# FeMTTU/femus

Hardware: AMD Instinct MI355X
Metric: assembled DOFs/sec + V-cycle SpMV GB/s (% HBM peak), 3D Poisson Q2 (higher is better)
Workload: dtype f64

## Files before the change

femus_amd/capi.py:

```python
import ctypes
import numpy as np
from ._lib import load_library

GEOM = {"hex": 0, "quad": 1, "line": 2, "tri": 3, "tet": 4, "wedge": 5}
FE = {"linear": 0, "serendipity": 1, "biquadratic": 2, "constant": 3, "pwlinear": 4}
GAUSS_ORDER = {"zero": 0, "first": 0, "second": 1, "third": 1, "fourth": 2, "fifth": 2,
               "sixth": 3, "seventh": 3, "eighth": 4, "ninth": 4}
OUTER = {"preonly": 0, "richardson": 1, "gmres": 2, "cg": 3, "fgmres": 4}
SMOOTH_JACOBI, SMOOTH_GS_COLOR, SMOOTH_VANKA, SMOOTH_SOR, SMOOTH_ILU0, SMOOTH_IDENTITY, SMOOTH_LU, SMOOTH_ASM = 0, 1, 2, 3, 4, 5, 6, 7


class FemusHipError(RuntimeError):
    pass


def _chk(rc):
    if rc != 0:
        raise FemusHipError(load_library().fh_last_error().decode())


def _i32(a):
    return np.ascontiguousarray(a, dtype=np.int32)


# ... 927 lines not shown
        a, g = ctypes.c_int(), ctypes.c_int()
        _chk(self.L.fh_assembler_affine_count(self.h, ctypes.byref(a), ctypes.byref(g)))
        return a.value, g.value

    def last_path(self):
        v = ctypes.c_int()
        _chk(self.L.fh_assembler_last_path(self.h, ctypes.byref(v)))
        return {1: "fused", 2: "two-pass"}.get(v.value)

    def fused_info(self):
        a, n, r = ctypes.c_int(), ctypes.c_int(), ctypes.c_int()
        pe = ctypes.c_int64()
        _chk(self.L.fh_assembler_fused_info(self.h, ctypes.byref(a), ctypes.byref(n), ctypes.byref(pe), ctypes.byref(r)))
        cs, ce = ctypes.c_int(), ctypes.c_int64()
        _chk(self.L.fh_assembler_carry_info(self.h, ctypes.byref(cs), ctypes.byref(ce)))
        return {"active": bool(a.value), "clusters": n.value, "partial_entries": pe.value, "second_pass_rows": r.value,
                "clusters_per_super": cs.value, "carried_entries": ce.value}

    def assemble_expr(self, A, res, sol, expr, scale=1.0):
        _chk(self.L.fh_assemble_poisson_expr(self.h, None if sol is None else sol.h, expr.h, float(scale), A.h, res.h))

    def element_matrices(self, sol=None, source_kind=0, params=(1.0,)):
        p = _f64(list(params) + [0.0] * (4 - len(params)))
        K, F = np.empty((self.nel, self.nc, self.nc)), np.empty((self.nel, self.nc))
        _chk(self.L.fh_element_matrices_poisson(self.h, None if sol is None else sol.h, int(source_kind), _p(p), _p(K), _p(F)))
        return K, F

    def info(self, colors=True):
        nco, by, fl = ctypes.c_int(), ctypes.c_int64(), ctypes.c_double()
        _chk(self.L.fh_assembler_info(self.h, ctypes.byref(nco) if colors else None, ctypes.byref(by), ctypes.byref(fl)))
        return {"ncolors": nco.value if colors else None, "algorithmic_bytes": by.value, "flops": fl.value}

# ... 400 lines not shown
```

femus_amd/csrc/fh_assemble.hip:

```cpp
#include "fh_internal.h"
#include "fh_fe.h"
#include "fh_expr_device.h"
#include <algorithm>

struct SfTab { double L[3][4], D[3][4]; };

struct fh_assembler_s {
  fh_ctx_t ctx = nullptr;
  int geom = 0, fe = 0, order = 0, dim = 3, nc = 27, ng = 64, nloc = 27;
  int nel = 0, nnode = 0, ndof = 0;
  int ncolors = 0;
  std::vector<int> color_ptr;
  int* d_color_elems = nullptr;
  int* d_elem_dof = nullptr;
  double* d_coords = nullptr;
  double* d_w = nullptr;
  double* d_phi = nullptr;
  double* d_dphi = nullptr;
  int* d_emap = nullptr;
  int* d_iota = nullptr;
  int ncp = 28;
  int* d_adj_ptr = nullptr;
  int* d_adj_ei = nullptr;
  unsigned char* d_rowmap = nullptr;
// ... 14 lines not shown
  bool kbuf_valid = false;
  bool rows_used_since = false;
  int last_path = 0;
  int cl_ncl = 0, cl_nm = 0, cl_ns = 0, cl_nprow = 0;
  int cl_sup_shift = 0;
  int cl_walk_shift = 0;
  size_t cl_ncarried = 0;
  size_t cl_npart = 0;
  unsigned* d_cl_sinfo = nullptr;
  void *d_cl_dtab = nullptr, *d_cl_fblk = nullptr, *d_cl_oblk = nullptr;
  int *d_cl_vdst = nullptr, *d_cl_fdst = nullptr;
  unsigned long long* d_cl_vdst64 = nullptr;
  double* cl_val_base = nullptr;
  unsigned char *d_cl_map = nullptr, *d_cl_pmap = nullptr;
  unsigned char* d_cl_mapb = nullptr;
  unsigned short* d_cl_gtab = nullptr;
  bool cl_all_rows = false;
  bool macro_valid = false;
  uint64_t macro_uid = 0;
  uint64_t macro_val_gen = 0;
  double* d_Pbuf = nullptr;
  int* d_cl_prow = nullptr;
  unsigned* d_cl_pstart = nullptr;
  int last_source_kind = 0;
  double last_params[2] = {1.0, 0.0};
  int *d_aff_elems = nullptr, *d_gen_elems = nullptr;
  int n_aff = 0, n_gen = 0;
  double *d_Mab = nullptr, *d_mphi = nullptr;
  double *d_mfT = nullptr, *d_mfPhi = nullptr;
  double* d_mfSFc = nullptr;
// ... 1587 lines not shown
static_assert(CL_ZC < (1 << 16), "cluster kernel: 16-bit double indices of the address blocks");
static_assert(cl_lds_bytes() <= 160 * 1024, "cluster kernel: LDS budget");
static_assert((CL_TAB % 2) == 0 && (CL_UVS % 2) == 0, "cluster kernel: 16-byte alignment of the wave regions");

struct ClParams {
  int ncl, ns, nm;
  int sup_shift;
  const uint2* dtab;
  const uint4* fblk;
  const uint4* oblk;
  const unsigned* sinfo;
  const unsigned long long* vdst;
  const int* fdst;
  const uint4* map;
  const uint4* mapb;
  double* Pbuf;
  double* res;
  unsigned long long* stamps;
};

__device__ __forceinline__ double cl_sum8(const char* S, const uint4 a, double t) {
  const unsigned w[4] = {a.x, a.y, a.z, a.w};
  double v[8];
#pragma unroll
  for (int k = 0; k < 8; k++) v[k] = *reinterpret_cast<const double*>(S + (((w[k >> 1] >> (16 * (k & 1))) & 0xffffu) << 3));
#pragma unroll
  for (int k = 0; k < 8; k++) t += v[k];
  return t;
}

// ... 49 lines not shown
  auto cl_at = [&](int it) {
    it = min(it, nit - 1);
    return ((((int)blockIdx.x + (it >> sh) * cstride)) << sh) + (it & ((1 << sh) - 1));
  };
  int cl = cl_at(0);
  {
    const int dof = P.elem_dof[(size_t)(cl * NW + wave) * P.nloc + nodeofl];
    if (lane < NC) {
      xt[lane] = P.coords[(size_t)dof * DIM];
      xt[28 + lane] = P.coords[(size_t)dof * DIM + 1];
      xt[56 + lane] = P.coords[(size_t)dof * DIM + 2];
      xt[84 + lane] = P.sol ? P.sol[dof] : 0.0;
    }
  }
  int dof_n = P.elem_dof[(size_t)(cl_at(1) * NW + wave) * P.nloc + nodeofl];
  wave_lds_sync();
  SfStamps st;
  if (INS) {
#pragma unroll
    for (int k = 0; k < 16; k++) st.acc[k] = 0;
    st.prev = __builtin_amdgcn_s_memtime();
  }
  int ndone = 0;
  double Dr[7];
  if (ahead) {
    sf_phase_a<SRC, REGC, INS>(P, LCl, CL_IDXA(), rcA, xt, UVa, Dr, &st);
    wave_lds_sync();
  }
#pragma unroll 1
  for (int it = 0; it < nit; it++) {
// ... 7 lines not shown
    const int cl_nn = cl_at(it + 2);
    const double nx0 = P.coords[(size_t)dof_n * DIM], nx1 = P.coords[(size_t)dof_n * DIM + 1], nx2 = P.coords[(size_t)dof_n * DIM + 2];
    const double nu = P.sol ? P.sol[dof_n] : 0.0;
    const int dof_nn = P.elem_dof[(size_t)(cl_nn * NW + wave) * P.nloc + nodeofl];
    double Kb[3][3], fsrc;
    if (!ahead) {
      sf_phase_a<SRC, REGC, INS>(P, LCl, CL_IDXA(), rcA, xt, UVa, Dr, &st);
      wave_lds_sync();
    }
    sf_stages<SRC, REGC, INS>(P, tab, LCl, LIl, rcZ, rcY, esym, ens, ensT, eout, R, lane, Dr, Kb, fsrc, &st);
    wave_lds_sync();
    sf_stamp<INS>(st, 6);
    const int tm = tid & (CL_NM_MAX - 1);
    const unsigned long long vd_cur = C.vdst[(size_t)cl * CL_NM_MAX + tm];
    const int fd_cur = C.fdst[(size_t)cl * CL_NM_MAX + tm];
    const uint4 mp_cur = C.map[(size_t)cl * CL_T + tid];
    const uint4 mq_cur = CARRY ? C.mapb[(size_t)cl * CL_T + tid] : make_uint4(0u, 0u, 0u, 0u);
    const int fv_own = CARRY ? C.fdst[(size_t)cl * CL_NM_MAX + wave * 16 + (lane & 15)] : 0;
    unsigned sinfo[CL_SPT];
#pragma unroll
    for (int i = 0; i < CL_SPT; i++) sinfo[i] = C.sinfo[i * CL_T + tid];
    double* Ks = R;
    {
      const bool diag = ((pk0 >> 29) & 1u) != 0;
      double* kd = Ks + (pk1 & 0xffffu);
      double* km = Ks + (pk1 >> 16);
#pragma unroll
      for (int a = 0; a < 3; a++)
#pragma unroll
        for (int a2 = 0; a2 < 3; a2++) {
          const double v = (a2 < a) ? (diag ? Kb[a2][a] : Kb[a][a2]) : Kb[a][a2];
          kd[a * 9 * KS + a2 * 9] = v;
          km[a2 * 9 * KS + a * 9] = v;
// ... 98 lines not shown
        cl_gdouble* dst = (cl_gdouble*)vb[i];
        if (P.debug & 64) *dst = vv[i];
        else if (!(P.debug & 4)) __builtin_nontemporal_store(vv[i], dst);
        else if (vv[i] == 1.2345e300) *dst = vv[i];
      }
      if (CARRY && lane < 16) {
        cl_gdouble* dst = (cl_gdouble*)(fvv < 0 ? C.Pbuf + (size_t)(fvv & 0x7fffffff) : C.res + (size_t)(fvv & 0x3fffffff));
        *dst = (fvv >= 0 && (fvv & 0x40000000)) ? fold + fsum : fsum;
      }
      sf_stamp<INS>(st, 15);
    }
    sf_stamp<INS>(st, 10);
    __syncthreads();
    sf_stamp<INS>(st, 11);
    dof_n = dof_nn;
    ndone++;
  }
  if (INS && C.stamps && lane == 0) {
    unsigned long long* o = C.stamps + ((size_t)blockIdx.x * NW + wave) * 20;
#pragma unroll
    for (int k = 0; k < 16; k++) o[k] = st.acc[k];
    o[16] = (unsigned long long)ndone;
  }
}

constexpr int RP_Q = 7;
template <int NT>
__global__ __launch_bounds__(256) void k_rows_partial(int nprow, const int* __restrict__ prow, const unsigned* __restrict__ pstart, const unsigned char* __restrict__ pmap,
                                                      const double* __restrict__ Pbuf, const int* __restrict__ rowptr, double* __restrict__ val, double* __restrict__ res, int nt) {
  __shared__ double acc[8][2][128];
// ... 211 lines not shown
  unsigned off = rowbase[g];
  int prev = -1;
  for (int a = aptr[g]; a < aptr[g + 1]; a++) {
    const int ei = aei[a], e = ei >> 5, cc = e / CL_NE;
    if (cc >= c) break;
    if (cc != prev) {
      prev = cc;
      const int r2 = T.tm[e % CL_NE][T.tof[ei & 31]];
      off += (unsigned)(T.roff[r2 + 1] - T.roff[r2]) + 1u;
    }
  }
  vdst[q] = (int)(0x80000000u | off);
  fdst[q] = (int)(0x80000000u | (off + (unsigned)(T.roff[r + 1] - T.roff[r])));
}

static int cluster_plan_build(fh_assembler_t as, fh_mat_t A, const int* elem_dof, const std::vector<int>& aptr, bool allow_carry = true) {
  fh_ctx_t ctx = as->ctx;
  const int nel = as->nel, nloc = as->nloc, m = A->m, KS = MF_KS;
  int nodeof[27];
  for (int n = 0; n < 27; n++) nodeof[(fhfe::xc(as->geom, n, 0) + 1) * 9 + (fhfe::xc(as->geom, n, 1) + 1) * 3 + fhfe::xc(as->geom, n, 2) + 1] = n;
  if (nel < CL_NE || nel % CL_NE || A->max_row > 128 || A->h_rowptr.empty()) return 0;
  const int ncl = nel / CL_NE;
  int tm[CL_NE][27], nm = 0;
  {
    std::vector<int> seen;
    for (int e = 0; e < CL_NE; e++)
      for (int t = 0; t < 27; t++) {
        const int g = elem_dof[(size_t)e * nloc + nodeof[t]];
        int k = -1;
        for (int q = 0; q < (int)seen.size(); q++)
// ... 224 lines not shown
    hipLaunchKernelGGL(k_cluster_maps, dim3(ncl), dim3(256), 0, ctx->stream, ncl, ns, nm, d_cdof, as->d_cl_sinfo, d_roff, d_tcol, as->d_cl_vdst, m, A->d_rowptr, A->d_col, d_complete,
                       as->d_adj_ptr, as->d_adj_ei, as->d_elem_dof, nloc, reinterpret_cast<uint4*>(as->d_cl_map), reinterpret_cast<uint4*>(as->d_cl_mapb), as->d_cl_pmap, d_first, d_err);
    if (sup_shift > 0 && m > 0)
      hipLaunchKernelGGL(k_cl_cover, dim3(fh_div_up(m, 256)), dim3(256), 0, ctx->stream, m, A->d_rowptr, d_complete, d_first, d_err, d_ncar);
    FH_CHECK_HIP(hipGetLastError());
    int err = 0;
    unsigned long long ncar = 0;
    FH_CHECK_HIP(hipMemcpyAsync(&err, d_err, sizeof(int), hipMemcpyDeviceToHost, ctx->stream));
    FH_CHECK_HIP(hipMemcpyAsync(&ncar, d_ncar, sizeof(ncar), hipMemcpyDeviceToHost, ctx->stream));
    FH_CHECK_HIP(hipStreamSynchronize(ctx->stream));
    as->cl_ncarried = (size_t)ncar;
    for (void* q : {(void*)d_tcol, (void*)d_roff, (void*)d_err}) hipFree(q);
    if (err && sup_shift > 0) {
      FH_TRACE("fh_assembler_create: carried rows do not cover their CSR rows -- cluster plan without them");
      for (void** q : {(void**)&as->d_cl_dtab, (void**)&as->d_cl_fblk, (void**)&as->d_cl_sinfo, (void**)&as->d_cl_oblk, (void**)&as->d_cl_gtab, (void**)&as->d_cl_vdst, (void**)&as->d_cl_vdst64,
                       (void**)&as->d_cl_fdst, (void**)&as->d_cl_map, (void**)&as->d_cl_mapb, (void**)&as->d_cl_pmap, (void**)&as->d_Pbuf, (void**)&as->d_cl_prow, (void**)&as->d_cl_pstart}) {
        if (*q) FH_CHECK_HIP(hipFree(*q));
        *q = nullptr;
      }
      return cluster_plan_build(as, A, elem_dof, aptr, false);
    }
    if (err) {
      FH_TRACE("fh_assembler_create: cluster maps could not be placed in the matrix pattern -- two-pass assembly kept");
      return 0;
    }
  }
  as->cl_ncl = ncl;
  as->cl_nm = nm;
  as->cl_ns = ns;
  as->cl_npart = npart;
  as->cl_nprow = (int)prow.size();
  as->cl_sup_shift = sup_shift;
  if (sup_shift > 0 || ctx->assemble_carry < 100) as->cl_walk_shift = sup_shift;
  as->fused = true;
  FH_TRACE("fh_assembler_create: cluster plan (%d clusters, %d macro nodes, %d entries; super-clusters of %d: %zu carried entries; %zu partial entries, %d rows in the second pass)", ncl,
           nm, ns, 1 << sup_shift, as->cl_ncarried, npart, as->cl_nprow);
  return 0;
}

template <bool CARRY>
static int launch_cluster_stamped(fh_assembler_t as, const AsmParams& P, const ClParams& C0, int grid) {
// ... 61 lines not shown
  out[k] = reinterpret_cast<unsigned long long>(v < 0 ? Pbuf + (size_t)(v & 0x7fffffff) : val + (size_t)v);
}

static int launch_cluster(fh_assembler_t as, const AsmParams& P, fh_mat_t A, double* res) {
  if (as->cl_val_base != A->d_val) {
    const size_t n = (size_t)as->cl_ncl * CL_NM_MAX;
    hipLaunchKernelGGL(k_cluster_vdst, dim3((unsigned)((n + 255) / 256)), dim3(256), 0, as->ctx->stream, n, as->d_cl_vdst, as->d_Pbuf, A->d_val, as->d_cl_vdst64);
    FH_CHECK_HIP(hipGetLastError());
    as->cl_val_base = A->d_val;
  }
  ClParams C;
  C.ncl = as->cl_ncl; C.ns = as->cl_ns; C.nm = as->cl_nm;
  C.dtab = reinterpret_cast<const uint2*>(as->d_cl_dtab); C.fblk = reinterpret_cast<const uint4*>(as->d_cl_fblk); C.oblk = reinterpret_cast<const uint4*>(as->d_cl_oblk);
  C.sinfo = as->d_cl_sinfo;
  C.vdst = as->d_cl_vdst64; C.fdst = as->d_cl_fdst; C.map = reinterpret_cast<const uint4*>(as->d_cl_map); C.mapb = reinterpret_cast<const uint4*>(as->d_cl_mapb);
  C.Pbuf = as->d_Pbuf; C.res = res;
  C.stamps = nullptr;
  C.sup_shift = as->cl_walk_shift;
  if (as->cl_sup_shift > 0 || (as->ctx->assemble_carry >= 200 && as->d_cl_mapb)) {
    if (P.source_kind == 4) FH_TRY((launch_cluster_one<2, true>(as, P, C)));
    else if (P.source_kind != 0) FH_TRY((launch_cluster_one<1, true>(as, P, C)));
    else FH_TRY((launch_cluster_one<0, true>(as, P, C)));
  } else if (P.source_kind == 4) FH_TRY((launch_cluster_one<2, false>(as, P, C)));
  else if (P.source_kind != 0) FH_TRY((launch_cluster_one<1, false>(as, P, C)));
  else FH_TRY((launch_cluster_one<0, false>(as, P, C)));
  if (as->cl_nprow > 0 && !(as->ctx->asm_debug & (2 | 8))) {
    if (!(as->ctx->asm_debug & 32))
      hipLaunchKernelGGL(k_rows_partial<0>, dim3(fh_div_up(as->cl_nprow, 16)), dim3(256), 0, as->ctx->stream, as->cl_nprow, as->d_cl_prow, as->d_cl_pstart,
                         as->d_cl_pmap, as->d_Pbuf, A->d_rowptr, A->d_val, res, 0);
    else
// ... 624 lines not shown
extern "C" int fh_assembler_destroy(fh_assembler_t as) {
  if (!as) return 0;
  hipStreamSynchronize(as->ctx->stream);
  if (as->d_color_elems) hipFree(as->d_color_elems);
  hipFree(as->d_elem_dof);
  hipFree(as->d_coords);
  hipFree(as->d_w);
  hipFree(as->d_phi);
  hipFree(as->d_dphi);
  if (as->d_emap) hipFree(as->d_emap);
  for (void* q : {(void*)as->d_aff_elems, (void*)as->d_gen_elems, (void*)as->d_Mab, (void*)as->d_mphi, (void*)as->d_mfT, (void*)as->d_mfPhi, (void*)as->d_mfSFc, (void*)as->d_mfSFi, (void*)as->d_sfLc, (void*)as->d_sfLi})
    if (q) hipFree(q);
  if (as->d_prog) hipFree(as->d_prog);
  if (as->d_prog_consts) hipFree(as->d_prog_consts);
  hipFree(as->d_iota);
  for (void* q : {(void*)as->d_cl_dtab, (void*)as->d_cl_fblk, (void*)as->d_cl_sinfo, (void*)as->d_cl_oblk, (void*)as->d_cl_gtab, (void*)as->d_cl_vdst, (void*)as->d_cl_vdst64, (void*)as->d_cl_fdst, (void*)as->d_cl_map, (void*)as->d_cl_mapb, (void*)as->d_cl_pmap,
                  (void*)as->d_Pbuf, (void*)as->d_cl_prow, (void*)as->d_cl_pstart})
    if (q) hipFree(q);
  for (void* q : {(void*)as->d_adj_ptr, (void*)as->d_adj_ei, (void*)as->d_rowmap, (void*)as->d_Kbuf, (void*)as->d_Fbuf, (void*)as->d_slot, (void*)as->d_gal_child,
                  (void*)as->d_gal_cnt, (void*)as->d_gal_row, (void*)as->d_gal_fb, (void*)as->d_gal_cb, (void*)as->d_gal_val, (void*)as->d_gal_res, (void*)as->d_gal_dense,
                  (void*)as->d_gal_fmask})
    if (q) hipFree(q);
  delete as;
  return 0;
}

static int assemble_poisson_core(fh_assembler_t as, fh_vec_t sol, int source_kind, const double* params, fh_mat_t A, fh_vec_t res);

extern "C" int fh_assemble_poisson(fh_assembler_t as, fh_vec_t sol, int source_kind, const double* params, fh_mat_t A, fh_vec_t res) {
  FH_REQUIRE(source_kind >= 0 && source_kind <= 3, "fh_assemble_poisson: unknown source kind %d", source_kind);
  return assemble_poisson_core(as, sol, source_kind, params, A, res);
// ... 172 lines not shown
  if (active) *active = on ? 1 : 0;
  if (nclusters) *nclusters = as->fused ? as->cl_ncl : 0;
  if (partial_entries) *partial_entries = as->fused ? (int64_t)as->cl_npart : 0;
  if (second_pass_rows) *second_pass_rows = as->fused ? as->cl_nprow : 0;
  return 0;
}

extern "C" int fh_assembler_carry_info(fh_assembler_t as, int* clusters_per_super, int64_t* carried_entries) {
  FH_REQUIRE(as, "fh_assembler_carry_info: null argument");
  const bool on = as->fused && as->ctx->assemble_fused && as->ctx->assemble_sf;
  if (clusters_per_super) *clusters_per_super = on ? 1 << as->cl_sup_shift : 0;
  if (carried_entries) *carried_entries = on ? (int64_t)as->cl_ncarried : 0;
  return 0;
}

extern "C" int fh_assembler_info(fh_assembler_t as, int* ncolors, int64_t* algorithmic_bytes, double* flops) {
  if (ncolors) {
    FH_TRY(ensure_colors(as));
    *ncolors = as->ncolors;
  }
  const int nc = as->nc, dim = as->dim, ng = as->ng;
  if (algorithmic_bytes) *algorithmic_bytes = (int64_t)as->nel * (nc * dim * 8 + nc * 4 + nc * 8 + nc * nc * 8 + nc * 8);
  if (flops)
    *flops = (double)as->nel * ng * (nc * dim * dim * 2.0 + 60.0 + nc * dim * dim * 2.0 + (double)nc * nc * (dim * 2.0 + 2.0) + nc * 10.0);
  return 0;
}

template <int NC, int NCH>
__global__ __launch_bounds__(256) void k_galerkin_elem(int nelc, const int* __restrict__ child, const int* __restrict__ slot_f, const double* __restrict__ Kf, int ks_f,
                                                       const int* __restrict__ edof_f, int nloc_f, const unsigned char* __restrict__ fb,
// ... 224 lines not shown
  if (k >= nelc * 9) return;
  const int E = k / 9, j = k % 9;
  unsigned m = 0;
  if (j < 8) {
    const int ej = child[(size_t)E * 8 + j];
    for (int n = 0; n < 27; n++) m |= (fb[edof_f[(size_t)ej * nloc_f + n]] ? 1u : 0u) << n;
    fmask[(size_t)E * 8 + j] = m;
  } else {
    for (int n = 0; n < 27; n++) m |= (cb[edof_c[(size_t)E * nloc_c + n]] ? 1u : 0u) << n;
    cmask[E] = m;
  }
}

template <bool INS>
__global__ __launch_bounds__(GMAC_T) void k_galerkin_macro(int nelc, const int* __restrict__ child, int nm, const unsigned* __restrict__ sinfo, const uint4* __restrict__ map,
                                                           const uint4* __restrict__ mapb , const unsigned long long* __restrict__ vdst, const unsigned short* __restrict__ gtab,
                                                           const unsigned* __restrict__ fmask, const unsigned* __restrict__ cmask,
                                                           const int* __restrict__ slot_c, double* __restrict__ Kc, int ks_c, const double* __restrict__ Cdense ,
                                                           unsigned long long* __restrict__ stamps) {
  constexpr int NC = 27, NCH = 8, NE = NC * NC, MT = 2, NK = GMAC_KP / 4;
  SfStamps st;
  if (INS) {
#pragma unroll
    for (int k = 0; k < 16; k++) st.acc[k] = 0;
  }
  extern __shared__ __attribute__((aligned(16))) double gmac_smem[];
  double* Tm = gmac_smem;
  unsigned long long* rbl = reinterpret_cast<unsigned long long*>(gmac_smem + GMAC_BUF);
  int* slds = reinterpret_cast<int*>(rbl + CL_NM_MAX);
  const int tid = threadIdx.x, lane = tid & 63, wave = __builtin_amdgcn_readfirstlane(tid >> 6);
  const int kk = lane >> 4, li = lane & 15;
// ... 5 lines not shown
#pragma unroll
  for (int m = 0; m < NK; m++)
#pragma unroll
    for (int x = 0; x < MT; x++) {
      const int r = 4 * m + kk, c = x * 16 + li;
      creg[m][x] = (r < NC && c < NC) ? Cdense[((size_t)wave * NC + r) * NC + c] : 0.0;
      const unsigned short g = (c < NC && r < NC) ? gtab[(size_t)wave * NE + c * NC + r] : (unsigned short)0xffff;
      gidx[m][x] = g == 0xffff ? -1 : (int)g;
    }
  typedef double d4 __attribute__((ext_vector_type(4)));
  const int stride = gridDim.x;
  int E = blockIdx.x;
  if (E >= nelc) return;
  const int tm = tid & (CL_NM_MAX - 1);
  int cl = child[(size_t)E * NCH] >> 3;
  if (tid < CL_NM_MAX) rbl[tid] = vdst[(size_t)cl * CL_NM_MAX + tm];
  uint4 mp = map[(size_t)cl * CL_T + tid];
  __syncthreads();
  double tv[CL_SPT];
  auto slot_pos = [&](const uint4& q4, int i) {
    const unsigned mq[4] = {q4.x, q4.y, q4.z, q4.w};
    const int r = si[i] & 127, p = (si[i] >> 7) & 127;
    if (r >= nm) return -1;
    if (!mapb) return p;
    return ((mq[2] >> (16 + i)) & 1u) ? -1 : (int)((mq[i >> 2] >> (8 * (i & 3))) & 255);
  };
  const uint4 qzero = make_uint4(0u, 0u, 0u, 0u);
  uint4 mq = mapb ? mapb[(size_t)cl * CL_T + tid] : qzero;
#pragma unroll
  for (int i = 0; i < CL_SPT; i++) {
    const int r = si[i] & 127, pos = slot_pos(mq, i);
    tv[i] = pos >= 0 ? reinterpret_cast<const double*>(rbl[r])[pos] : 0.0;
  }
  int En = min(E + stride, nelc - 1);
  int cln = child[(size_t)En * NCH] >> 3;
  unsigned long long vdn = vdst[(size_t)cln * CL_NM_MAX + tm];
  uint4 mpn = map[(size_t)cln * CL_T + tid];
  uint4 mqn = mapb ? mapb[(size_t)cln * CL_T + tid] : qzero;
  const int ln = min(lane, NC - 1);
  unsigned dmask = fmask[(size_t)E * NCH + wave], cdm = cmask[E];
  int slc = slot_c[(size_t)E * NC + ln];
  if (INS) st.prev = __builtin_amdgcn_s_memtime();
  int ndone = 0;
#pragma unroll 1
  for (; E < nelc; E += stride) {
    sf_stamp<INS>(st, 0);
    {
      const unsigned mw[4] = {mp.x, mp.y, mp.z, mp.w};
#pragma unroll
      for (int i = 0; i < CL_SPT; i++) {
        const int r = si[i] & 127, j = (mw[i >> 2] >> (8 * (i & 3))) & 255;
        if (r < nm) Tm[(si[i] >> 14) + j] = tv[i];
      }
// ... 2 lines not shown
    if (tid < NC) slds[tid] = slc;
    sf_stamp<INS>(st, 1);
    __syncthreads();
    sf_stamp<INS>(st, 2);
    mp = mpn;
    mq = mqn;
#pragma unroll
    for (int i = 0; i < CL_SPT; i++) {
      const int r = si[i] & 127, pos = slot_pos(mq, i);
      tv[i] = pos >= 0 ? reinterpret_cast<const double*>(rbl[r])[pos] : 0.0;
    }
    {
      const int Enn = min(E + 2 * stride, nelc - 1);
      const int clnn = child[(size_t)Enn * NCH] >> 3;
      vdn = vdst[(size_t)clnn * CL_NM_MAX + tm];
      mpn = map[(size_t)clnn * CL_T + tid];
      if (mapb) mqn = mapb[(size_t)clnn * CL_T + tid];
    }
    const unsigned long long cdead = cdm, dead = dmask;
    {
      const int En1 = min(E + stride, nelc - 1);
      dmask = fmask[(size_t)En1 * NCH + wave];
      cdm = cmask[En1];
      slc = slot_c[(size_t)En1 * NC + ln];
    }
    sf_stamp<INS>(st, 3);
    d4 T[MT][MT], KE[MT][MT];
#pragma unroll
    for (int a = 0; a < MT; a++)
#pragma unroll
      for (int b = 0; b < MT; b++) { T[a][b] = d4{0.0, 0.0, 0.0, 0.0}; KE[a][b] = d4{0.0, 0.0, 0.0, 0.0}; }
    {
// ... 177 lines not shown
  const int grid = std::max(1, std::min(fh_div_up(cas->nel, 4), c->num_cu * 2));
  if (from_macro) {
    static bool attr_set_m[64] = {};
    if (!attr_set_m[c->device & 63]) {
      FH_CHECK_HIP(hipFuncSetAttribute(reinterpret_cast<const void*>(&k_galerkin_macro<false>), hipFuncAttributeMaxDynamicSharedMemorySize, (int)gmac_lds_bytes()));
      FH_CHECK_HIP(hipFuncSetAttribute(reinterpret_cast<const void*>(&k_galerkin_macro<true>), hipFuncAttributeMaxDynamicSharedMemorySize, (int)gmac_lds_bytes()));
      attr_set_m[c->device & 63] = true;
    }
    const int gm_grid = std::max(1, std::min(cas->nel, c->num_cu));
    if (c->asm_debug & 128) {
      unsigned long long* d_st = nullptr;
      const size_t nst = (size_t)gm_grid * GMAC_NW * 20;
      FH_CHECK_HIP(hipMalloc(&d_st, nst * sizeof(unsigned long long)));
      FH_CHECK_HIP(hipMemsetAsync(d_st, 0, nst * sizeof(unsigned long long), c->stream));
      hipLaunchKernelGGL(k_galerkin_macro<true>, dim3(gm_grid), dim3(GMAC_T), gmac_lds_bytes(), c->stream, cas->nel, cas->d_gal_child, fas->cl_nm, fas->d_cl_sinfo,
                         reinterpret_cast<const uint4*>(fas->d_cl_map), reinterpret_cast<const uint4*>(fas->d_cl_mapb), fas->d_cl_vdst64, fas->d_cl_gtab, cas->d_gal_fmask, cas->d_gal_fmask + (size_t)cas->nel * 8, cas->d_slot, cas->d_Kbuf,
                         cas->kstride, cas->d_gal_dense, d_st);
      std::vector<unsigned long long> h(nst);
      FH_CHECK_HIP(hipMemcpyAsync(h.data(), d_st, nst * sizeof(unsigned long long), hipMemcpyDeviceToHost, c->stream));
      FH_CHECK_HIP(hipStreamSynchronize(c->stream));
      FH_CHECK_HIP(hipFree(d_st));
      static const char* name[10] = {"loop top", "macro matrix into LDS", "barrier", "next cluster's loads issued, look-ups", "K~ fragments gathered, two products (56 MFMA)",
                                     "barrier (all waves done with the macro matrix)", "result into LDS", "barrier", "eight results added, coarse rows stored", "barrier"};
      double sum[10] = {0}, ncl = 0, tot = 0;
      for (size_t w = 0; w < (size_t)gm_grid * GMAC_NW; w++) {
        for (int k = 0; k < 10; k++) sum[k] += (double)h[w * 20 + k];
        ncl += (double)h[w * 20 + 16];
      }
      for (int k = 0; k < 10; k++) tot += sum[k];
      fprintf(stderr, "k_galerkin_macro phase stamps: %.0f shader-clock ticks per cluster and wave\n", tot / std::max(ncl, 1.0));
      for (int k = 0; k < 10; k++) fprintf(stderr, "  %2d %-62s %9.1f  %5.1f %%\n", k, name[k], sum[k] / std::max(ncl, 1.0), 100.0 * sum[k] / std::max(tot, 1.0));
    } else
      hipLaunchKernelGGL(k_galerkin_macro<false>, dim3(gm_grid), dim3(GMAC_T), gmac_lds_bytes(), c->stream, cas->nel, cas->d_gal_child, fas->cl_nm, fas->d_cl_sinfo,
                         reinterpret_cast<const uint4*>(fas->d_cl_map), reinterpret_cast<const uint4*>(fas->d_cl_mapb), fas->d_cl_vdst64, fas->d_cl_gtab, cas->d_gal_fmask, cas->d_gal_fmask + (size_t)cas->nel * 8, cas->d_slot, cas->d_Kbuf,
                         cas->kstride, cas->d_gal_dense, (unsigned long long*)nullptr);
  } else if (c->galerkin_mfma) {
    const size_t lds = nc == 27 ? galerkin_mfma_lds<27, 8>() : galerkin_mfma_lds<9, 4>();
    static bool attr_set[64] = {};
    if (!attr_set[c->device & 63]) {
      FH_CHECK_HIP(hipFuncSetAttribute(reinterpret_cast<const void*>(&k_galerkin_mfma<27, 8>), hipFuncAttributeMaxDynamicSharedMemorySize, (int)galerkin_mfma_lds<27, 8>()));
      FH_CHECK_HIP(hipFuncSetAttribute(reinterpret_cast<const void*>(&k_galerkin_mfma<9, 4>), hipFuncAttributeMaxDynamicSharedMemorySize, (int)galerkin_mfma_lds<9, 4>()));
      attr_set[c->device & 63] = true;
    }
    const int g1 = std::max(1, std::min(fh_div_up(cas->nel, GAL_NW), c->num_cu));
    if (nc == 27)
      hipLaunchKernelGGL((k_galerkin_mfma<27, 8>), dim3(g1), dim3(GAL_NW * 64), lds, c->stream, cas->nel, cas->d_gal_child, fas->d_slot, fas->d_Kbuf, fas->kstride, fas->d_elem_dof,
                         fas->nloc, cas->d_gal_fb, cas->d_slot, cas->d_Kbuf, cas->kstride, cas->d_elem_dof, cas->nloc, cas->d_gal_cb, cas->d_gal_dense);
    else
      hipLaunchKernelGGL((k_galerkin_mfma<9, 4>), dim3(g1), dim3(GAL_NW * 64), lds, c->stream, cas->nel, cas->d_gal_child, fas->d_slot, fas->d_Kbuf, fas->kstride, fas->d_elem_dof,
// ... 19 lines not shown
```

femus_amd/csrc/fh_core.hip:

```cpp
#include <cstdlib>
#include "fh_internal.h"
#include <chrono>
#include <cstdlib>
#include <cstdarg>
#include <cmath>

static thread_local char g_err[1024] = "";

void fh_set_error(const char* fmt, ...) {
  va_list ap;
  va_start(ap, fmt);
  vsnprintf(g_err, sizeof(g_err), fmt, ap);
  va_end(ap);
}

extern "C" const char* fh_last_error(void) { return g_err; }

bool fh_trace_on() {
  static const bool on = [] {
    const char* e = getenv("FEMUS_HIP_TRACE");
    return e && *e && *e != '0';
  }();
  return on;
}
// ... 201 lines not shown
  else if (!strcmp(name, "vanka_persistent")) c->vanka_persistent = (int)value;
  else if (!strcmp(name, "coarse_reduce")) c->coarse_reduce = (int)value;
  else if (!strcmp(name, "coarse_nd")) c->coarse_nd = (int)value;
  else if (!strcmp(name, "coarse_nd_min")) c->coarse_nd_min = (int)value;
  else if (!strcmp(name, "coarse_direct")) c->coarse_direct = (int)value;
  else if (!strcmp(name, "gmres_device")) c->gmres_device = (int)value;
  else if (!strcmp(name, "galerkin_macro")) c->galerkin_macro = (int)value;
  else if (!strcmp(name, "vanka_fused")) c->vanka_fused = (int)value;
  else if (!strcmp(name, "coarse_direct_min")) c->coarse_direct_min = (int)value;
  else if (!strcmp(name, "coarse_nd_streams")) c->coarse_nd_streams = (int)value;
  else if (!strcmp(name, "patch_invert_lds")) c->patch_invert_lds = (int)value;
  else if (!strcmp(name, "gj_mfma")) c->gj_mfma = (int)value;
  else if (!strcmp(name, "gj_symmetric")) c->gj_symmetric = (int)value;
  else if (!strcmp(name, "assemble_affine")) c->assemble_affine = (int)value;
  else if (!strcmp(name, "assemble_carry")) c->assemble_carry = (int)value;
  else if (!strcmp(name, "tri_runs")) c->tri_runs = (int)value;
  else if (!strcmp(name, "ilu_ahead")) c->ilu_ahead = (int)value;
  else if (!strcmp(name, "use_graph")) c->use_graph = (int)value;
  else if (!strcmp(name, "mg_reuse_graph")) c->mg_reuse_graph = (int)value;
  else if (!strcmp(name, "spgemm_slot_map")) c->spgemm_slot_map = (int)value;
  else if (!strcmp(name, "device_setup")) c->device_setup = (int)value;
  else if (!strcmp(name, "spgemm_device_symbolic")) c->spgemm_device_symbolic = (int)value;
  else if (!strcmp(name, "halo_overlap")) c->halo_overlap = (int)value;
  else if (!strcmp(name, "halo_profile")) c->halo_profile = (int)value;
  else if (!strcmp(name, "halo_self_rccl")) c->halo_self_rccl = (int)value;
  else {
    fh_set_error("fh_set_option: unknown option '%s'", name);
    return 2;
  }
  return 0;
// ... 325 lines not shown
```

femus_amd/csrc/fh_internal.h:

```cpp
#pragma once
#include <hip/hip_runtime.h>
#include <cstdint>
#include <cstdio>
#include <cstdlib>
#include <cstring>
#include <new>
#include <stdexcept>
#include <string>
#include <algorithm>
#include <vector>
#include "../../include/femus_hip.h"

void fh_set_error(const char* fmt, ...);

#define FH_CHECK_HIP(expr)                                                                        \
  do {                                                                                            \
    hipError_t _e = (expr);                                                                       \
    if (_e != hipSuccess) {                                                                       \
      fh_set_error("%s:%d: %s failed: %s", __FILE__, __LINE__, #expr, hipGetErrorString(_e));     \
      return 1;                                                                                   \
    }                                                                                             \
  } while (0)

#define FH_REQUIRE(cond, ...)                                                                     \
// ... 56 lines not shown
  int debug_poison = 0;
  int assemble_mfma = 12;
  int assemble_rows_nt = 1;
  int assemble_sf_grid = 1;
  int assemble_sf = 8;
  int assemble_sumfac = 1;
  int assemble_rows2 = 1;
  int generic_pack = 1;
  int assemble_kpad = 1;
  int assemble_sym = 1;
  int assemble_two_pass = 1;
  int assemble_fused = 1;
  int ilu_ahead = 2;
  int tri_runs = 1;
  int assemble_carry = -1;
  int assemble_affine = 0;
  int gj_symmetric = 1;
  int galerkin_mfma = 1;
  int patch_invert_lds = 1;
  int coarse_nd = 8;
  int coarse_nd_streams = 0;
  int coarse_nd_min = 1024;
  int vanka_fused = 1;
  int galerkin_macro = 1;
  int gmres_device = 1;
  int coarse_direct = 1;
  int coarse_direct_min = 8192;
  int coarse_reduce = 1;
  int vanka_persistent = 0;
  int gj_block = 128;
// ... 130 lines not shown
```

include/femus_hip.h:

```cpp
#ifndef FEMUS_HIP_H
#define FEMUS_HIP_H

#include <stddef.h>
#include <stdint.h>

#ifdef __cplusplus
extern "C" {
#endif

typedef struct fh_ctx_s* fh_ctx_t;
typedef struct fh_vec_s* fh_vec_t;
typedef struct fh_mat_s* fh_mat_t;
typedef struct fh_mg_s* fh_mg_t;
typedef struct fh_mesh_s* fh_mesh_t;
typedef struct fh_halo_s* fh_halo_t;
typedef struct fh_graph_s* fh_graph_t;

int fh_device_count(int* n);
int fh_init(int device, fh_ctx_t* ctx);
int fh_finalize(fh_ctx_t ctx);
const char* fh_last_error(void);
const char* fh_version(void);
int fh_device_name(fh_ctx_t ctx, char* buf, int buflen);
int fh_sync(fh_ctx_t ctx);
// ... 115 lines not shown
int fh_mesh_amr_constraints(fh_mesh_t mesh, int fe, int* n_hanging, int* nnz, int* hanging, int* ptr, int* master, double* weight);
int fh_build_amr_prolongator(fh_ctx_t ctx, fh_mesh_t mesh, int fe, fh_mat_t* P_amr);

typedef struct fh_assembler_s* fh_assembler_t;
int fh_assembler_create(fh_ctx_t ctx, int geom, int fe, int gauss_order, int nel, int nloc, const int* elem_dof,
                        int nnode, const double* coords , fh_mat_t A, fh_assembler_t* as);
int fh_assembler_create_mesh(fh_ctx_t ctx, fh_mesh_t mesh, int fe, int gauss_order, fh_mat_t A, fh_assembler_t* as);
int fh_assembler_destroy(fh_assembler_t as);
int fh_assembler_galerkin(fh_assembler_t fine, fh_assembler_t coarse, const int* child, int nfb, const int* fbdc, int ncb, const int* cbdc, fh_mat_t Ac);
int fh_assemble_poisson(fh_assembler_t as, fh_vec_t sol, int source_kind, const double* params, fh_mat_t A, fh_vec_t res);
int fh_assembler_info(fh_assembler_t as, int* ncolors, int64_t* algorithmic_bytes, double* flops);
int fh_element_matrices_poisson(fh_assembler_t as, fh_vec_t sol, int source_kind, const double* params, double* K, double* F);
int fh_assembler_affine_count(fh_assembler_t as, int* n_affine, int* n_general);
int fh_assembler_fused_info(fh_assembler_t as, int* active, int* nclusters, int64_t* partial_entries, int* second_pass_rows);
int fh_assembler_carry_info(fh_assembler_t as, int* clusters_per_super, int64_t* carried_entries);
int fh_assembler_last_path(fh_assembler_t as, int* path);

int fh_fe_face_nodes(int geom, int fe, int face, int* nfn, int* local_nodes);
int fh_fe_node_ref(int geom, int node, int* xi );
int fh_fe_node_ref_coords(int geom, int node, double* xi );
int fh_assemble_neumann_faces(fh_ctx_t ctx, int geom, int fe, int gauss_order, int nfaces, const int* face_nodes, const double* tau,
                              int nnode, const double* coords, fh_vec_t res);

typedef struct fh_expr_s* fh_expr_t;
int fh_expr_compile(const char* expression, const char* variables, fh_expr_t* expr);
int fh_expr_eval(fh_expr_t expr, const double* x, double* value);
int fh_expr_eval_many(fh_expr_t expr, int npts, const double* x , double* values);
int fh_expr_eval_device(fh_ctx_t ctx, fh_expr_t expr, int npts, const double* x , double* values);
int fh_expr_program(fh_expr_t expr, int* ncode, int* nconst, int* code , double* consts );
int fh_expr_nvars(fh_expr_t expr, int* nvars);
// ... 134 lines not shown
```

Measured before the change: 814.9 million.

## Deduplicate per-cluster scatter map words into shared classes

At assembler setup, clusters whose map and mapb words are identical are grouped: the words are hashed on device, matched by hash on the host, checked for exact equality, and then one copy per class is gathered. The fused cluster kernel and the Galerkin macro kernel then look up a class index through a small indirection table instead of reading a full per-cluster map. This is meant to cut the bytes the assembly kernel streams per cluster (16 or 32 bytes per thread) and let the shared tables stay in cache, in exchange for an extra scalar load per cluster and a longer setup. Sharing only happens when there are at most a quarter as many classes as clusters, and it is on by default.

```diff
diff --git a/femus_amd/capi.py b/femus_amd/capi.py
--- a/femus_amd/capi.py
+++ b/femus_amd/capi.py
@@ -965,8 +965,10 @@
         _chk(self.L.fh_assembler_fused_info(self.h, ctypes.byref(a), ctypes.byref(n), ctypes.byref(pe), ctypes.byref(r)))
         cs, ce = ctypes.c_int(), ctypes.c_int64()
         _chk(self.L.fh_assembler_carry_info(self.h, ctypes.byref(cs), ctypes.byref(ce)))
+        pc, pb = ctypes.c_int(), ctypes.c_int64()
+        _chk(self.L.fh_assembler_plan_info(self.h, ctypes.byref(pc), ctypes.byref(pb)))
         return {"active": bool(a.value), "clusters": n.value, "partial_entries": pe.value, "second_pass_rows": r.value,
-                "clusters_per_super": cs.value, "carried_entries": ce.value}
+                "clusters_per_super": cs.value, "carried_entries": ce.value, "plan_classes": pc.value, "plan_bytes_per_cluster": pb.value}
 
     def assemble_expr(self, A, res, sol, expr, scale=1.0):
         _chk(self.L.fh_assemble_poisson_expr(self.h, None if sol is None else sol.h, expr.h, float(scale), A.h, res.h))
diff --git a/femus_amd/csrc/fh_assemble.hip b/femus_amd/csrc/fh_assemble.hip
--- a/femus_amd/csrc/fh_assemble.hip
+++ b/femus_amd/csrc/fh_assemble.hip
@@ -2,6 +2,7 @@
 #include "fh_fe.h"
 #include "fh_expr_device.h"
 #include <algorithm>
+#include <unordered_map>
 
 struct SfTab { double L[3][4], D[3][4]; };
 
@@ -52,6 +53,8 @@
   double* cl_val_base = nullptr;
   unsigned char *d_cl_map = nullptr, *d_cl_pmap = nullptr;
   unsigned char* d_cl_mapb = nullptr;
+  int* d_cl_ccls = nullptr;
+  int cl_ncls = 0;
   unsigned short* d_cl_gtab = nullptr;
   bool cl_all_rows = false;
   bool macro_valid = false;
@@ -1669,6 +1672,7 @@
   const int* fdst;
   const uint4* map;
   const uint4* mapb;
+  const int* ccls;
   double* Pbuf;
   double* res;
   unsigned long long* stamps;
@@ -1748,6 +1752,10 @@
     }
   }
   int dof_n = P.elem_dof[(size_t)(cl_at(1) * NW + wave) * P.nloc + nodeofl];
+  typedef __attribute__((address_space(4))) const int cl_cint;
+  auto blk_at = [&](int c) { return C.ccls ? *(cl_cint*)(C.ccls + c) : c; };
+  int blk = blk_at(cl);
+  asm volatile("" : "+s"(blk));
   wave_lds_sync();
   SfStamps st;
   if (INS) {
@@ -1785,9 +1793,10 @@
     const int tm = tid & (CL_NM_MAX - 1);
     const unsigned long long vd_cur = C.vdst[(size_t)cl * CL_NM_MAX + tm];
     const int fd_cur = C.fdst[(size_t)cl * CL_NM_MAX + tm];
-    const uint4 mp_cur = C.map[(size_t)cl * CL_T + tid];
-    const uint4 mq_cur = CARRY ? C.mapb[(size_t)cl * CL_T + tid] : make_uint4(0u, 0u, 0u, 0u);
+    const uint4 mp_cur = C.map[(size_t)blk * CL_T + tid];
+    const uint4 mq_cur = CARRY ? C.mapb[(size_t)blk * CL_T + tid] : make_uint4(0u, 0u, 0u, 0u);
     const int fv_own = CARRY ? C.fdst[(size_t)cl * CL_NM_MAX + wave * 16 + (lane & 15)] : 0;
+    int blk_n = blk_at(cl_at(it + 1));
     unsigned sinfo[CL_SPT];
 #pragma unroll
     for (int i = 0; i < CL_SPT; i++) sinfo[i] = C.sinfo[i * CL_T + tid];
@@ -1916,6 +1925,8 @@
     __syncthreads();
     sf_stamp<INS>(st, 11);
     dof_n = dof_nn;
+    asm volatile("" : "+s"(blk_n));
+    blk = blk_n;
     ndone++;
   }
   if (INS && C.stamps && lane == 0) {
@@ -2157,6 +2168,106 @@
   fdst[q] = (int)(0x80000000u | (off + (unsigned)(T.roff[r + 1] - T.roff[r])));
 }
 
+__device__ __forceinline__ unsigned long long cl_mix64(unsigned long long x) {
+  x = (x ^ (x >> 30)) * 0xbf58476d1ce4e5b9ull;
+  x = (x ^ (x >> 27)) * 0x94d049bb133111ebull;
+  return x ^ (x >> 31);
+}
+__global__ __launch_bounds__(256) void k_cl_hash(const uint4* __restrict__ map, const uint4* __restrict__ mapb , unsigned long long* __restrict__ hash) {
+  __shared__ unsigned long long acc;
+  const int c = blockIdx.x;
+  if (threadIdx.x == 0) acc = 0;
+  __syncthreads();
+  unsigned long long h = 0;
+  for (int t = threadIdx.x; t < CL_T; t += 256)
+    for (int b = 0; b < (mapb ? 2 : 1); b++) {
+      const uint4 w = (b ? mapb : map)[(size_t)c * CL_T + t];
+      const unsigned long long k = (unsigned long long)(4 * t + 2 * b + 1) * 0x9e3779b97f4a7c15ull;
+      h += cl_mix64((((unsigned long long)w.y << 32) | w.x) + k) + cl_mix64((((unsigned long long)w.w << 32) | w.z) + k + 0x9e3779b97f4a7c15ull);
+    }
+  atomicAdd(&acc, h);
+  __syncthreads();
+  if (threadIdx.x == 0) hash[c] = acc;
+}
+__global__ __launch_bounds__(256) void k_cl_same(const uint4* __restrict__ map, const uint4* __restrict__ mapb , int* __restrict__ rep) {
+  __shared__ int differs;
+  const int c = blockIdx.x, r = rep[c];
+  if (r == c) return;
+  if (threadIdx.x == 0) differs = 0;
+  __syncthreads();
+  bool d = false;
+  for (int t = threadIdx.x; t < CL_T; t += 256)
+    for (int b = 0; b < (mapb ? 2 : 1); b++) {
+      const uint4 x = (b ? mapb : map)[(size_t)c * CL_T + t], y = (b ? mapb : map)[(size_t)r * CL_T + t];
+      d = d || x.x != y.x || x.y != y.y || x.z != y.z || x.w != y.w;
+    }
+  if (d) differs = 1;
+  __syncthreads();
+  if (threadIdx.x == 0 && differs) rep[c] = c;
+}
+__global__ __launch_bounds__(256) void k_cl_gather(const int* __restrict__ first , const uint4* __restrict__ src, uint4* __restrict__ dst) {
+  const size_t k = blockIdx.x, c = (size_t)first[k];
+  for (int t = threadIdx.x; t < CL_T; t += 256) dst[k * CL_T + t] = src[c * CL_T + t];
+}
+static int cluster_plan_share(fh_assembler_t as, int ncl) {
+  fh_ctx_t ctx = as->ctx;
+  const uint4* map = reinterpret_cast<const uint4*>(as->d_cl_map);
+  const uint4* mapb = reinterpret_cast<const uint4*>(as->d_cl_mapb);
+  struct Tmp {
+    std::vector<void*> p;
+    ~Tmp() { for (void* q : p) if (q) hipFree(q); }
+  } tmp;
+  unsigned long long* d_hash = nullptr;
+  int *d_rep = nullptr, *d_first = nullptr;
+  FH_CHECK_HIP(hipMalloc(&d_hash, (size_t)ncl * sizeof(unsigned long long)));
+  tmp.p.push_back(d_hash);
+  FH_CHECK_HIP(hipMalloc(&d_rep, (size_t)ncl * sizeof(int)));
+  tmp.p.push_back(d_rep);
+  hipLaunchKernelGGL(k_cl_hash, dim3(ncl), dim3(256), 0, ctx->stream, map, mapb, d_hash);
+  FH_CHECK_HIP(hipGetLastError());
+  std::vector<unsigned long long> hash(ncl);
+  FH_CHECK_HIP(hipMemcpyAsync(hash.data(), d_hash, (size_t)ncl * sizeof(unsigned long long), hipMemcpyDeviceToHost, ctx->stream));
+  FH_CHECK_HIP(hipStreamSynchronize(ctx->stream));
+  std::vector<int> rep(ncl);
+  {
+    std::unordered_map<unsigned long long, int> seen;
+    seen.reserve((size_t)ncl);
+    for (int c = 0; c < ncl; c++) rep[c] = seen.emplace(hash[c], c).first->second;
+  }
+  FH_CHECK_HIP(hipMemcpyAsync(d_rep, rep.data(), (size_t)ncl * sizeof(int), hipMemcpyHostToDevice, ctx->stream));
+  hipLaunchKernelGGL(k_cl_same, dim3(ncl), dim3(256), 0, ctx->stream, map, mapb, d_rep);
+  FH_CHECK_HIP(hipGetLastError());
+  FH_CHECK_HIP(hipMemcpyAsync(rep.data(), d_rep, (size_t)ncl * sizeof(int), hipMemcpyDeviceToHost, ctx->stream));
+  FH_CHECK_HIP(hipStreamSynchronize(ctx->stream));
+  std::vector<int> first, ccls(ncl, -1);
+  for (int c = 0; c < ncl; c++)
+    if (rep[c] == c) { ccls[c] = (int)first.size(); first.push_back(c); }
+  for (int c = 0; c < ncl; c++) ccls[c] = ccls[rep[c]];
+  const int ncls = (int)first.size();
+  as->cl_ncls = ncls;
+  if ((size_t)ncls * 4 > (size_t)ncl) {
+    FH_TRACE("fh_assembler_create: cluster plan: %d classes of map words for %d clusters -- a copy per cluster kept", ncls, ncl);
+    return 0;
+  }
+  FH_CHECK_HIP(hipMalloc(&d_first, (size_t)ncls * sizeof(int)));
+  tmp.p.push_back(d_first);
+  FH_CHECK_HIP(hipMemcpyAsync(d_first, first.data(), (size_t)ncls * sizeof(int), hipMemcpyHostToDevice, ctx->stream));
+  for (unsigned char** arr : {&as->d_cl_map, &as->d_cl_mapb}) {
+    if (!*arr) continue;
+    unsigned char* tab = nullptr;
+    FH_CHECK_HIP(hipMalloc(&tab, (size_t)ncls * CL_T * 16));
+    hipLaunchKernelGGL(k_cl_gather, dim3(ncls), dim3(256), 0, ctx->stream, d_first, reinterpret_cast<const uint4*>(*arr), reinterpret_cast<uint4*>(tab));
+    FH_CHECK_HIP(hipStreamSynchronize(ctx->stream));
+    FH_CHECK_HIP(hipFree(*arr));
+    *arr = tab;
+  }
+  FH_CHECK_HIP(hipGetLastError());
+  FH_CHECK_HIP(hipMalloc(&as->d_cl_ccls, (size_t)ncl * sizeof(int)));
+  FH_CHECK_HIP(hipMemcpy(as->d_cl_ccls, ccls.data(), (size_t)ncl * sizeof(int), hipMemcpyHostToDevice));
+  FH_TRACE("fh_assembler_create: cluster plan: %d classes of map words for %d clusters", ncls, ncl);
+  return 0;
+}
+
 static int cluster_plan_build(fh_assembler_t as, fh_mat_t A, const int* elem_dof, const std::vector<int>& aptr, bool allow_carry = true) {
   fh_ctx_t ctx = as->ctx;
   const int nel = as->nel, nloc = as->nloc, m = A->m, KS = MF_KS;
@@ -2411,7 +2522,7 @@
     if (err && sup_shift > 0) {
       FH_TRACE("fh_assembler_create: carried rows do not cover their CSR rows -- cluster plan without them");
       for (void** q : {(void**)&as->d_cl_dtab, (void**)&as->d_cl_fblk, (void**)&as->d_cl_sinfo, (void**)&as->d_cl_oblk, (void**)&as->d_cl_gtab, (void**)&as->d_cl_vdst, (void**)&as->d_cl_vdst64,
-                       (void**)&as->d_cl_fdst, (void**)&as->d_cl_map, (void**)&as->d_cl_mapb, (void**)&as->d_cl_pmap, (void**)&as->d_Pbuf, (void**)&as->d_cl_prow, (void**)&as->d_cl_pstart}) {
+                       (void**)&as->d_cl_fdst, (void**)&as->d_cl_map, (void**)&as->d_cl_mapb, (void**)&as->d_cl_ccls, (void**)&as->d_cl_pmap, (void**)&as->d_Pbuf, (void**)&as->d_cl_prow, (void**)&as->d_cl_pstart}) {
         if (*q) FH_CHECK_HIP(hipFree(*q));
         *q = nullptr;
       }
@@ -2422,6 +2533,8 @@
       return 0;
     }
   }
+  as->cl_ncls = 0;
+  if (ctx->cluster_plan_classes) FH_TRY(cluster_plan_share(as, ncl));
   as->cl_ncl = ncl;
   as->cl_nm = nm;
   as->cl_ns = ns;
@@ -2513,6 +2626,7 @@
   C.dtab = reinterpret_cast<const uint2*>(as->d_cl_dtab); C.fblk = reinterpret_cast<const uint4*>(as->d_cl_fblk); C.oblk = reinterpret_cast<const uint4*>(as->d_cl_oblk);
   C.sinfo = as->d_cl_sinfo;
   C.vdst = as->d_cl_vdst64; C.fdst = as->d_cl_fdst; C.map = reinterpret_cast<const uint4*>(as->d_cl_map); C.mapb = reinterpret_cast<const uint4*>(as->d_cl_mapb);
+  C.ccls = as->d_cl_ccls;
   C.Pbuf = as->d_Pbuf; C.res = res;
   C.stamps = nullptr;
   C.sup_shift = as->cl_walk_shift;
@@ -3167,7 +3281,7 @@
   if (as->d_prog) hipFree(as->d_prog);
   if (as->d_prog_consts) hipFree(as->d_prog_consts);
   hipFree(as->d_iota);
-  for (void* q : {(void*)as->d_cl_dtab, (void*)as->d_cl_fblk, (void*)as->d_cl_sinfo, (void*)as->d_cl_oblk, (void*)as->d_cl_gtab, (void*)as->d_cl_vdst, (void*)as->d_cl_vdst64, (void*)as->d_cl_fdst, (void*)as->d_cl_map, (void*)as->d_cl_mapb, (void*)as->d_cl_pmap,
+  for (void* q : {(void*)as->d_cl_dtab, (void*)as->d_cl_fblk, (void*)as->d_cl_sinfo, (void*)as->d_cl_oblk, (void*)as->d_cl_gtab, (void*)as->d_cl_vdst, (void*)as->d_cl_vdst64, (void*)as->d_cl_fdst, (void*)as->d_cl_map, (void*)as->d_cl_mapb, (void*)as->d_cl_ccls, (void*)as->d_cl_pmap,
                   (void*)as->d_Pbuf, (void*)as->d_cl_prow, (void*)as->d_cl_pstart})
     if (q) hipFree(q);
   for (void* q : {(void*)as->d_adj_ptr, (void*)as->d_adj_ei, (void*)as->d_rowmap, (void*)as->d_Kbuf, (void*)as->d_Fbuf, (void*)as->d_slot, (void*)as->d_gal_child,
@@ -3370,6 +3484,16 @@
   return 0;
 }
 
+extern "C" int fh_assembler_plan_info(fh_assembler_t as, int* plan_classes, int64_t* plan_bytes_per_cluster) {
+  FH_REQUIRE(as, "fh_assembler_plan_info: null argument");
+  const bool on = as->fused && as->ctx->assemble_fused && as->ctx->assemble_sf;
+  const bool carry = as->cl_sup_shift > 0 || as->d_cl_mapb;
+  if (plan_classes) *plan_classes = on ? (as->cl_ncls ? as->cl_ncls : as->cl_ncl) : 0;
+  if (plan_bytes_per_cluster)
+    *plan_bytes_per_cluster = on ? (int64_t)(CL_NM_MAX * 8 + CL_NM_MAX * 4 + (carry ? CL_NE * 16 * 4 : 0)) + (as->d_cl_ccls ? 4 : (int64_t)CL_T * 16 * (carry ? 2 : 1)) : 0;
+  return 0;
+}
+
 extern "C" int fh_assembler_info(fh_assembler_t as, int* ncolors, int64_t* algorithmic_bytes, double* flops) {
   if (ncolors) {
     FH_TRY(ensure_colors(as));
@@ -3624,7 +3748,8 @@
 
 template <bool INS>
 __global__ __launch_bounds__(GMAC_T) void k_galerkin_macro(int nelc, const int* __restrict__ child, int nm, const unsigned* __restrict__ sinfo, const uint4* __restrict__ map,
-                                                           const uint4* __restrict__ mapb , const unsigned long long* __restrict__ vdst, const unsigned short* __restrict__ gtab,
+                                                           const uint4* __restrict__ mapb , const int* __restrict__ ccls ,
+                                                           const unsigned long long* __restrict__ vdst, const unsigned short* __restrict__ gtab,
                                                            const unsigned* __restrict__ fmask, const unsigned* __restrict__ cmask,
                                                            const int* __restrict__ slot_c, double* __restrict__ Kc, int ks_c, const double* __restrict__ Cdense ,
                                                            unsigned long long* __restrict__ stamps) {
@@ -3660,8 +3785,9 @@
   if (E >= nelc) return;
   const int tm = tid & (CL_NM_MAX - 1);
   int cl = child[(size_t)E * NCH] >> 3;
+  auto blk_of = [&](int c) { return ccls ? ccls[c] : c; };
   if (tid < CL_NM_MAX) rbl[tid] = vdst[(size_t)cl * CL_NM_MAX + tm];
-  uint4 mp = map[(size_t)cl * CL_T + tid];
+  uint4 mp = map[(size_t)blk_of(cl) * CL_T + tid];
   __syncthreads();
   double tv[CL_SPT];
   auto slot_pos = [&](const uint4& q4, int i) {
@@ -3672,7 +3798,7 @@
     return ((mq[2] >> (16 + i)) & 1u) ? -1 : (int)((mq[i >> 2] >> (8 * (i & 3))) & 255);
   };
   const uint4 qzero = make_uint4(0u, 0u, 0u, 0u);
-  uint4 mq = mapb ? mapb[(size_t)cl * CL_T + tid] : qzero;
+  uint4 mq = mapb ? mapb[(size_t)blk_of(cl) * CL_T + tid] : qzero;
 #pragma unroll
   for (int i = 0; i < CL_SPT; i++) {
     const int r = si[i] & 127, pos = slot_pos(mq, i);
@@ -3681,8 +3807,8 @@
   int En = min(E + stride, nelc - 1);
   int cln = child[(size_t)En * NCH] >> 3;
   unsigned long long vdn = vdst[(size_t)cln * CL_NM_MAX + tm];
-  uint4 mpn = map[(size_t)cln * CL_T + tid];
-  uint4 mqn = mapb ? mapb[(size_t)cln * CL_T + tid] : qzero;
+  uint4 mpn = map[(size_t)blk_of(cln) * CL_T + tid];
+  uint4 mqn = mapb ? mapb[(size_t)blk_of(cln) * CL_T + tid] : qzero;
   const int ln = min(lane, NC - 1);
   unsigned dmask = fmask[(size_t)E * NCH + wave], cdm = cmask[E];
   int slc = slot_c[(size_t)E * NC + ln];
@@ -3715,8 +3841,9 @@
       const int Enn = min(E + 2 * stride, nelc - 1);
       const int clnn = child[(size_t)Enn * NCH] >> 3;
       vdn = vdst[(size_t)clnn * CL_NM_MAX + tm];
-      mpn = map[(size_t)clnn * CL_T + tid];
-      if (mapb) mqn = mapb[(size_t)clnn * CL_T + tid];
+      const int bnn = blk_of(clnn);
+      mpn = map[(size_t)bnn * CL_T + tid];
+      if (mapb) mqn = mapb[(size_t)bnn * CL_T + tid];
     }
     const unsigned long long cdead = cdm, dead = dmask;
     {
@@ -3924,7 +4051,7 @@
       FH_CHECK_HIP(hipMalloc(&d_st, nst * sizeof(unsigned long long)));
       FH_CHECK_HIP(hipMemsetAsync(d_st, 0, nst * sizeof(unsigned long long), c->stream));
       hipLaunchKernelGGL(k_galerkin_macro<true>, dim3(gm_grid), dim3(GMAC_T), gmac_lds_bytes(), c->stream, cas->nel, cas->d_gal_child, fas->cl_nm, fas->d_cl_sinfo,
-                         reinterpret_cast<const uint4*>(fas->d_cl_map), reinterpret_cast<const uint4*>(fas->d_cl_mapb), fas->d_cl_vdst64, fas->d_cl_gtab, cas->d_gal_fmask, cas->d_gal_fmask + (size_t)cas->nel * 8, cas->d_slot, cas->d_Kbuf,
+                         reinterpret_cast<const uint4*>(fas->d_cl_map), reinterpret_cast<const uint4*>(fas->d_cl_mapb), fas->d_cl_ccls, fas->d_cl_vdst64, fas->d_cl_gtab, cas->d_gal_fmask, cas->d_gal_fmask + (size_t)cas->nel * 8, cas->d_slot, cas->d_Kbuf,
                          cas->kstride, cas->d_gal_dense, d_st);
       std::vector<unsigned long long> h(nst);
       FH_CHECK_HIP(hipMemcpyAsync(h.data(), d_st, nst * sizeof(unsigned long long), hipMemcpyDeviceToHost, c->stream));
@@ -3942,7 +4069,7 @@
       for (int k = 0; k < 10; k++) fprintf(stderr, "  %2d %-62s %9.1f  %5.1f %%\n", k, name[k], sum[k] / std::max(ncl, 1.0), 100.0 * sum[k] / std::max(tot, 1.0));
     } else
       hipLaunchKernelGGL(k_galerkin_macro<false>, dim3(gm_grid), dim3(GMAC_T), gmac_lds_bytes(), c->stream, cas->nel, cas->d_gal_child, fas->cl_nm, fas->d_cl_sinfo,
-                         reinterpret_cast<const uint4*>(fas->d_cl_map), reinterpret_cast<const uint4*>(fas->d_cl_mapb), fas->d_cl_vdst64, fas->d_cl_gtab, cas->d_gal_fmask, cas->d_gal_fmask + (size_t)cas->nel * 8, cas->d_slot, cas->d_Kbuf,
+                         reinterpret_cast<const uint4*>(fas->d_cl_map), reinterpret_cast<const uint4*>(fas->d_cl_mapb), fas->d_cl_ccls, fas->d_cl_vdst64, fas->d_cl_gtab, cas->d_gal_fmask, cas->d_gal_fmask + (size_t)cas->nel * 8, cas->d_slot, cas->d_Kbuf,
                          cas->kstride, cas->d_gal_dense, (unsigned long long*)nullptr);
   } else if (c->galerkin_mfma) {
     const size_t lds = nc == 27 ? galerkin_mfma_lds<27, 8>() : galerkin_mfma_lds<9, 4>();
diff --git a/femus_amd/csrc/fh_core.hip b/femus_amd/csrc/fh_core.hip
--- a/femus_amd/csrc/fh_core.hip
+++ b/femus_amd/csrc/fh_core.hip
@@ -239,6 +239,7 @@
   else if (!strcmp(name, "gj_symmetric")) c->gj_symmetric = (int)value;
   else if (!strcmp(name, "assemble_affine")) c->assemble_affine = (int)value;
   else if (!strcmp(name, "assemble_carry")) c->assemble_carry = (int)value;
+  else if (!strcmp(name, "cluster_plan_classes")) c->cluster_plan_classes = (int)value;
   else if (!strcmp(name, "tri_runs")) c->tri_runs = (int)value;
   else if (!strcmp(name, "ilu_ahead")) c->ilu_ahead = (int)value;
   else if (!strcmp(name, "use_graph")) c->use_graph = (int)value;
diff --git a/femus_amd/csrc/fh_internal.h b/femus_amd/csrc/fh_internal.h
--- a/femus_amd/csrc/fh_internal.h
+++ b/femus_amd/csrc/fh_internal.h
@@ -94,6 +94,7 @@
   int ilu_ahead = 2;
   int tri_runs = 1;
   int assemble_carry = -1;
+  int cluster_plan_classes = 1;
   int assemble_affine = 0;
   int gj_symmetric = 1;
   int galerkin_mfma = 1;
diff --git a/include/femus_hip.h b/include/femus_hip.h
--- a/include/femus_hip.h
+++ b/include/femus_hip.h
@@ -153,6 +153,7 @@
 int fh_assembler_affine_count(fh_assembler_t as, int* n_affine, int* n_general);
 int fh_assembler_fused_info(fh_assembler_t as, int* active, int* nclusters, int64_t* partial_entries, int* second_pass_rows);
 int fh_assembler_carry_info(fh_assembler_t as, int* clusters_per_super, int64_t* carried_entries);
+int fh_assembler_plan_info(fh_assembler_t as, int* plan_classes, int64_t* plan_bytes_per_cluster);
 int fh_assembler_last_path(fh_assembler_t as, int* path);
 
 int fh_fe_face_nodes(int geom, int fe, int face, int* nfn, int* local_nodes);
```

Result: no change. 814.2 million (-0.1%).
